# Cogito2012/3DFaceRecon

Hardware: AMD Instinct MI355X
Metric: faces/sec (3DMM decode+depth render), batch 64 @200x200 (higher is better)
Workload: dtype f32

## Files before the change

### 3dfacerecon_amd/_lib.py

```python
import ctypes
import hashlib
import os
import shutil
import subprocess
import sys
import threading
import types

_PKG_DIR = os.path.dirname(os.path.abspath(__file__))
_CSRC = os.path.join(_PKG_DIR, "csrc")
LIB_PATH = os.path.join(_PKG_DIR, "libfr_hotpath.so")
SOURCES = ["fr_capi.hip", "fr_render.hip", "fr_decode.hip", "fr_decode_q.hip", "fr_decode_bwd.hip", "fr_render_bwd.hip", "fr_render_nbwd.hip",
           "fr_render_tbwd.hip", "fr_sfs.hip", "fr_depth_normals.hip", "fr_geometry.hip", "fr_fine_losses.hip", "fr_depth_interp.hip",
           "fr_albedo_lse.hip", "fr_synth.hip", "fr_photo.hip", "fr_mesh.hip", "fr_coverage.hip", "fr_landmark.hip",
           "fr_landmark_solve.hip", "fr_landmark_contour.hip", "fr_photo_solve.hip", "fr_attr_interp.hip"]
HEADERS = [os.path.join(_CSRC, "fr_common.h"), os.path.join(_CSRC, "fr_decode_shared.h"), os.path.join(_CSRC, "fr_sfs_pinv.h"),
           os.path.join(_CSRC, "fr_owner_scatter.h"), os.path.join(_CSRC, "fr_shade.h"), os.path.join(_CSRC, "fr_landmark_shared.h"),
           os.path.join(_CSRC, "fr_point_weight.h"),
           os.path.join(_PKG_DIR, "..", "include", "fr_hotpath.h")]
HIPCC_FLAGS = ["--offload-arch=gfx950", "-O3", "-std=c++17", "-ffp-contract=off", "-fPIC", "-shared",
               "-mllvm", "-amdgpu-atomic-optimizer-strategy=None"]

FR_OK = 0
_ERR_NAMES = {-1: "invalid argument", -2: "workspace / packed buffer too small", -3: "HIP launch or runtime error",
# ... 147 lines not shown
    "fr_fine_losses_backward":                        "i:ppppiiippp",
    "fr_debug_fine_losses_geom":                      "v:iiiI",
    "fr_depth_interp_forward":                        "i:pippiiiiipp",
    "fr_depth_interp_backward_workspace_bytes":       "z:iiii",
    "fr_depth_interp_backward":                       "i:ppipppiiiiiipzp",
    "fr_debug_depth_interp_bwd_geom":                 "v:iiiiI",
    "fr_albedo_basis_bytes":                          "z:ii",
    "fr_albedo_basis_build":                          "i:ppiiipzp",
    "fr_sfs_lighting":                                "i:piiidpzp",
    "fr_albedo_lse_workspace_bytes":                  "z:iiii",
    "fr_albedo_lse_forward":                          "i:ppppppiiiiidppppzp",
    "fr_debug_albedo_lse_geom":                       "v:iiiiI",
    "fr_synth_params":                                "i:uuiiiifffpppppp",
    "fr_synth_texture":                               "i:pppiiipp",
    "fr_synth_shade":                                 "i:pppppiiiiffppp",
    "fr_synth_texture_backward_workspace_bytes":      "z:iii",
    "fr_synth_texture_backward":                      "i:ppiiippzp",
    "fr_photo_loss_state_bytes":                      "z:iii",
    "fr_photo_loss_forward":                          "i:ppppppiiiffppzp",
    "fr_photo_loss_backward":                         "i:ppppppppiiiffpppp",
    "fr_debug_photo_loss_geom":                       "v:iiiI",
    "fr_synth_light_rgb":                             "i:uuippp",
    "fr_synth_shade_rgb":                             "i:pppppiiiiffpppp",
    "fr_photo_loss_rgb_state_bytes":                  "z:iii",
    "fr_photo_loss_rgb_forward":                      "i:ppppppiiiffppzp",
    "fr_photo_loss_rgb_backward":                     "i:ppppppppiiiffpppp",
    "fr_debug_photo_loss_rgb_geom":                   "v:iiiI",
    "fr_albedo_basis_rgb_bytes":                      "z:ii",
    "fr_albedo_basis_rgb_build":                      "i:pppiiipzp",
    "fr_albedo_image_rgb":                            "i:pppiiiiipp",
    "fr_photo_solve_rgb_workspace_bytes":             "z:iii",
    "fr_photo_light_lse_rgb_forward":                 "i:ppppppiiiffdppppzp",
    "fr_albedo_lse_rgb_forward":                      "i:ppppppiiiiiffdppppzp",
    "fr_debug_photo_solve_rgb_geom":                  "v:iiiI",
    "fr_mesh_visible":                                "i:ppiiiiipp",
    "fr_mesh_lift":                                   "i:pippppiiiiipipp",
    "fr_mesh_vertex_normals":                         "i:pipppiiipip",
    "fr_attr_interp_forward":                         "i:pipippiiiiipp",
    "fr_attr_interp_backward":                        "i:ppipipppipiiiiiippp",
    "fr_mesh_vertex_normals_backward":                "i:pipipppiiippiip",
    "fr_debug_attr_interp_bwd_geom":                  "v:iiiiI",
    "fr_coverage_forward":                            "i:pippiiiiipp",
    "fr_coverage_backward_workspace_bytes":           "z:iiii",
    "fr_coverage_backward":                           "i:pppipppiiiiiipzp",
    "fr_debug_coverage_bwd_geom":                     "v:iiiiI",
    "fr_landmark_basis_bytes":                        "z:iii",
    "fr_landmark_basis_build":                        "i:ppppiiiipzp",
    "fr_landmark_forward":                            "i:ppzpppiiiiifppp",
    "fr_landmark_backward":                           "i:ppppzpppiiiiifppip",
    "fr_landmark_solve_workspace_bytes":              "z:iii",
    "fr_landmark_solve_step":                         "i:ppzppipppiiiiiifppppzp",
    "fr_landmark_contour_select":                     "i:ppzpppippipiiiiiiifppppp",
    "fr_debug_render_geom":                           "v:iiiiiI",
    "fr_debug_decode_bwd_geom":                       "v:iiiiI",
    "fr_debug_decode_geom":                           "i:iiiiiI",
    "fr_debug_decode_q_geom":                         "i:iiiiiiI",
    "fr_debug_decode_walk":                           "i:iiiiI",
    "fr_debug_pose_bwd_geom":                         "v:iiI",
    "fr_debug_render_bwd_geom":                       "v:iiiiI",
    "fr_debug_div3_sweep":                            "i:uupp",
    "fr_debug_clock_probe":                           "i:piip",
}
EXPORTS = list(SIGNATURES)


def bind(cdll, names=None):
    for name in (SIGNATURES if names is None else names):
        ret, args = SIGNATURES[name].split(":")
        fn = getattr(cdll, name)
        fn.restype = _CTYPE[ret]
        fn.argtypes = [_CTYPE[c] for c in args]
    return cdll


def lib():
    global _lib
    if _lib is None:
        with _lock:
            if _lib is None:
                import torch
                if is_stale():
                    compile()
                try:
                    L = bind(ctypes.CDLL(LIB_PATH))
                except OSError as e:
                    raise RuntimeError("fr_hotpath: cannot load %s (%s); run compile() -- there is no CPU fallback"
                                       % (LIB_PATH, e))
                want = src_hash()
                if want is not None and want.encode() not in L.fr_version():
                    raise RuntimeError("fr_hotpath: %s reports %r but the sources hash to %s: stale binary refused"
                                       % (LIB_PATH, L.fr_version(), want))
                _lib = L
    return _lib


DECODE_ARITH_Q30, DECODE_ARITH_F32 = 0, 1
_STATE = sys.modules.setdefault("_fr_hotpath_state", types.SimpleNamespace(decode_arith=None, q30_levels=7, option_epoch=0,
                                                                           pools={}))
_ARITH_ENV = {"q30": 7, "q30l7": 7, "q30l5": 5, "q30l4": 4}


def _torch_stream_key(dev):
    import torch
    return (dev.index if dev.index is not None else torch.cuda.current_device(), torch.cuda.current_stream(dev).cuda_stream,
            torch.cuda.is_current_stream_capturing())

# ... 159 lines not shown
```

### 3dfacerecon_amd/csrc/fr_capi.hip

```cpp
#include <atomic>
#include <mutex>

#include "fr_common.h"
#include "fr_landmark_shared.h"

namespace {
struct OptDesc {
    const char* name;
    int dflt;
    const char* word;
};
const OptDesc kOpts[fr::OPT_COUNT] = {
    {"FR_DECODE_IMPL", 0, "loop"}, {"FR_DECODE_WIDE", 1, nullptr}, {"FR_DECODE_NBW", 0, nullptr},
    {"FR_DECODE_WAVES", 16, nullptr}, {"FR_DECODE_NT", -1, nullptr}, {"FR_RESOLVE_OPT", 2, nullptr},
    {"FR_EMIT_FILTER", 3, nullptr}, {"FR_RENDER_IMPL", 0, "scan"}, {"FR_RESOLVE_BLOCK", 0, nullptr},
    {"FR_RENDER_ROWS", 0, nullptr}, {"FR_DECODE_STORE", 0, nullptr},
    {"FR_BWD_CHUNKS", 256, nullptr}, {"FR_BWD_CB", 0, nullptr}, {"FR_EMIT_ORDER", -1, nullptr},
    {"FR_Q30_SCHED", 0, nullptr}, {"FR_DECODE_CUS", 0, nullptr},
};
std::atomic<int> g_opt[fr::OPT_COUNT];
std::once_flag g_opt_once;
void opts_init() {
    for (int i = 0; i < fr::OPT_COUNT; i++) {
        int v = kOpts[i].dflt;
        const char* e = getenv(kOpts[i].name);
        if (e && *e) v = (kOpts[i].word && !strcmp(e, kOpts[i].word)) ? 1 : atoi(e);
        g_opt[i].store(v, std::memory_order_relaxed);
    }
}
int opt_index(const char* name) {
    if (!name) return -1;
    for (int i = 0; i < fr::OPT_COUNT; i++)
        if (!strcmp(name, kOpts[i].name)) return i;
    return -1;
}
}

int fr::opt(fr::Opt o) {
    std::call_once(g_opt_once, opts_init);
    return g_opt[o].load(std::memory_order_relaxed);
}

extern "C" {

int fr_set_option(const char* name, int value) {
    const int i = opt_index(name);
    if (i < 0) return FR_ERR_INVALID_ARG;
    std::call_once(g_opt_once, opts_init);
    g_opt[i].store(value, std::memory_order_relaxed);
    return FR_OK;
}

int fr_get_option(const char* name, int* value) {
    const int i = opt_index(name);
    if (i < 0 || !value) return FR_ERR_INVALID_ARG;
    *value = fr::opt((fr::Opt)i);
    return FR_OK;
}

#ifndef FR_SRC_HASH
#define FR_SRC_HASH "unhashed"
#endif
const char* fr_version(void) { return "fr_hotpath 0.4 (gfx950) src=" FR_SRC_HASH; }

const char* fr_strerror(int code) {
    switch (code) {
        case FR_OK: return "ok";
        case FR_ERR_INVALID_ARG: return "invalid argument";
        case FR_ERR_WORKSPACE: return "workspace / packed buffer too small";
        case FR_ERR_LAUNCH: return "HIP launch or runtime error";
        case FR_ERR_UNSUPPORTED: return "size not supported by the gfx950 kernels";
// ... 583 lines not shown
```

### 3dfacerecon_amd/csrc/fr_common.h

```cpp
#pragma once
#include <hip/hip_runtime.h>
#include <atomic>
#include <limits.h>
#include <stdint.h>
#include <stdlib.h>
#include <string.h>

#include "../../include/fr_hotpath.h"

namespace fr {

__device__ __forceinline__ float bg_depth() { return -99999999999999.0f; }

__device__ __forceinline__ int f2i_x86(float f) {
    return (f >= -2147483648.0f && f < 2147483648.0f) ? (int)f : INT_MIN;
}

__device__ __forceinline__ float mn(float a, float b) { return a < b ? a : b; }
__device__ __forceinline__ float mx(float a, float b) { return a > b ? a : b; }

__device__ __forceinline__ uint32_t f32_ord(float h) {
    uint32_t u = __float_as_uint(h);
    return (u & 0x80000000u) ? ~u : (u | 0x80000000u);
}
// ... 54 lines not shown

template <int K>
__device__ __forceinline__ double row_shl_f64(double v) {
    int lo = __double2loint(v), hi = __double2hiint(v);
    lo = __builtin_amdgcn_update_dpp(0, lo, 0x100 + K, 0xF, 0xF, true);
    hi = __builtin_amdgcn_update_dpp(0, hi, 0x100 + K, 0xF, 0xF, true);
    return __hiloint2double(hi, lo);
}
__device__ __forceinline__ double wave_tree_f64(double v) {
    v = v + __shfl_down(v, 32u, 64);
    v = v + __shfl_down(v, 16u, 64);
    v = v + row_shl_f64<8>(v);
    v = v + row_shl_f64<4>(v);
    v = v + row_shl_f64<2>(v);
    v = v + row_shl_f64<1>(v);
    return v;
}

}

typedef std::atomic<unsigned char> fr_lds_flags_t;
inline hipError_t fr_allow_full_lds(const void* kernel, fr_lds_flags_t* done ) {
    int dev = 0;
    hipError_t e = hipGetDevice(&dev);
    if (e != hipSuccess) return e;
    if (dev >= 0 && dev < 64 && done[dev].load(std::memory_order_acquire)) return hipSuccess;
    e = hipFuncSetAttribute(kernel, hipFuncAttributeMaxDynamicSharedMemorySize, 160 * 1024);
    if (e == hipSuccess && dev >= 0 && dev < 64) done[dev].store(1, std::memory_order_release);
    return e;
}

inline bool ws_ok(const void* p, size_t have, size_t need, size_t align) {
    return p && !((uintptr_t)p & (align - 1)) && have >= need;
}

namespace fr {
enum Opt {
    OPT_DECODE_IMPL,
    OPT_DECODE_WIDE,
    OPT_DECODE_NBW,
    OPT_DECODE_WAVES,
    OPT_DECODE_NT,
    OPT_RESOLVE_OPT,
    OPT_EMIT_FILTER,
    OPT_RENDER_IMPL,
    OPT_RESOLVE_BLOCK,
    OPT_RENDER_ROWS,
    OPT_DECODE_STORE,
    OPT_BWD_CHUNKS,
    OPT_BWD_CB,
    OPT_EMIT_ORDER,
    OPT_Q30_SCHED,
    OPT_DECODE_CUS,
    OPT_COUNT
};
int opt(Opt o);
}

int fr_launch_render_forward(const float* vertex, const float* tri, const float* texture, int B, int nver, int ntri,
                             int H, int W, int tex_batch, float* depth, float* tex_img, float* normal,
                             float* tri_ind, void* workspace, size_t ws_bytes, hipStream_t stream);
int fr_launch_render_forward_phases(const float* vertex, const float* tri, const float* texture, int B, int nver, int ntri,
                                    int H, int W, int tex_batch, float* depth, float* tex_img, float* normal,
                                    float* tri_ind, void* workspace, size_t ws_bytes, hipStream_t stream, int phases,
                                    long long vpitch = 0, int rows_hint = 0);
int fr_launch_rendering_layer(const float* vertex, const float* tri, const float* texture, const float* im_gray, int B,
                              int nver, int ntri, int H, int W, int tex_batch, float* net_in, float* depth_img,
                              float* depth, float* tri_ind, void* workspace, size_t ws_bytes, hipStream_t stream, int phases = 7,
                              long long vpitch = 0, int rows_hint = 0);
bool fr_rendering_layer_supported(int B, int nver, int ntri, int H, int W);
int fr_launch_render_backward(const float* depth_grad, const float* tri, const float* tri_ind, float* vertex_grad,
                              int B, int nver, int ntri, int H, int W, void* workspace, size_t ws_bytes,
                              hipStream_t stream);
struct FrPixelGrad {
    const float* g_depth;
    const float* g_depth_img;
    const float* g_net_input;
    const float* im_gray;
    const float* depth;
};
int fr_launch_render_backward_z(const FrPixelGrad& pg, const float* tri, const float* tri_ind, float* zplane, int zpitch,
                                int B, int nver, int ntri, int H, int W, void* workspace, size_t ws_bytes, hipStream_t stream);
size_t fr_render_backward_workspace_bytes_impl(int B, int H, int W);
size_t fr_render_workspace_bytes_impl(int B, int ntri, int H, int W);
size_t fr_packed_basis_bytes(int N, int n_shape, int n_exp);
int fr_launch_pack_basis(const float* mu, const float* pc_shape, const float* pc_exp, int N, int n_shape, int n_exp,
                         void* packed, hipStream_t stream);
int fr_launch_decode(const float* params, const void* packed, const float* R_override, int B, int N, int n_shape,
                     int n_exp, float im_size, float* vertex_proj, int pitch, hipStream_t stream);
int fr_launch_clock_probe(unsigned long long* out, int blocks, int iters, hipStream_t stream);
size_t fr_packed_q_bytes(int N, int n_shape, int n_exp);
bool fr_decode_q_supported(int n_shape, int n_exp);
int fr_launch_pack_q(const float* mu, const float* pc_shape, const float* pc_exp, int N, int n_shape, int n_exp,
                     void* qimage, hipStream_t stream);
int fr_launch_decode_q(const float* params, const void* qimage, const float* R_override, int B, int N, int n_shape,
                       int n_exp, float im_size, float* vertex_proj, int pitch, int levels, void* workspace, size_t ws_bytes,
                       hipStream_t stream);
bool fr_decode_q_levels_ok(int levels);
size_t fr_decode_q_workspace_bytes_impl(int n_shape, int n_exp);
int fr_device_cu_count();
int fr_decode_plan_cus();
size_t fr_decode_backward_workspace_impl(int N, int ns, int ne);
int fr_launch_decode_backward(const float* grad_vertex_proj, const float* params, const float* vertex_proj,
                              const float* pc_shape, const float* pc_exp, const float* R_override, int B, int N, int ns,
                              int ne, float im_size, float* grad_params, void* workspace, hipStream_t stream,
                              const void* packed_t = nullptr, const float* mu = nullptr, int zpitch = 0);
// ... 37 lines not shown
```

### 3dfacerecon_amd/csrc/fr_render.hip

```cpp
#include "fr_common.h"
#include <stddef.h>

namespace fr {

struct alignas(64) RenderArgs {
    const float* vertex;
    long long face_stride_b;
    long long vpitch_b;
    const int4* tri4_lane;
    long long tex_stride;
    int nseg;
    uint32_t nseg_magic;
    uint32_t nseg_shift;
    int emit_q, emit_r;
    int strips;
    float wm1, hm1;
    int use_filter;
    int nver, ntri;
    uint32_t rows_magic;
    const float* texture;
    float4* tritex_ws;
    const int4* tri4;
    uint4* recs;
    uint16_t* segoff;
// ... 285 lines not shown
            float4* t4 = reinterpret_cast<float4*>(txi) + 3 * (size_t)g;
            t4[0] = make_float4(o[0].tex[0], o[0].tex[1], o[0].tex[2], o[1].tex[0]);
            t4[1] = make_float4(o[1].tex[1], o[1].tex[2], o[2].tex[0], o[2].tex[1]);
            t4[2] = make_float4(o[2].tex[2], o[3].tex[0], o[3].tex[1], o[3].tex[2]);
            float4* n4 = reinterpret_cast<float4*>(nrm) + 3 * (size_t)g;
            n4[0] = make_float4(o[0].nrm[0], o[0].nrm[1], o[0].nrm[2], o[1].nrm[0]);
            n4[1] = make_float4(o[1].nrm[1], o[1].nrm[2], o[2].nrm[0], o[2].nrm[1]);
            n4[2] = make_float4(o[2].nrm[2], o[3].nrm[0], o[3].nrm[1], o[3].nrm[2]);
        }
    } else {
        for (int i = tid; i < npix; i += BLOCK) {
            PixelOut o = resolve_pixel(keys[i], vx, vy, vz, tri, tex, nver, ntri);
            dep[i] = o.depth;
            tin[i] = o.tind;
#pragma unroll
            for (int j = 0; j < 3; j++) {
                txi[3 * (size_t)i + j] = o.tex[j];
                nrm[3 * (size_t)i + j] = o.nrm[j];
            }
        }
    }
}

template <int BLOCK>
__global__ __launch_bounds__(BLOCK) void render_strip_kernel(RenderArgs a) {
    extern __shared__ __attribute__((aligned(16))) unsigned long long keys[];
    const int tid = threadIdx.x;
    const int bin = xcd_remap(blockIdx.x, gridDim.x);
    const int b = bin / a.strips;
    const int s = bin - b * a.strips;
    const int r0 = s * a.rows;
    const int r1 = min(a.H, r0 + a.rows);
    const int npix = (r1 - r0) * a.W;
    const unsigned long long KBG = bg_key();
    for (int i = tid; i < npix; i += BLOCK) keys[i] = KBG;
    __syncthreads();
    const float* __restrict__ vx = a.vertex + (size_t)b * 3 * a.vpitch;
    const float* __restrict__ vy = vx + a.vpitch;
    const float* __restrict__ vz = vy + a.vpitch;
    for (int t = tid; t < a.ntri; t += BLOCK)
        raster_triangle_into_strip(t, a.tri, vx, vy, vz, a.nver, a.ntri, a.H, a.W, r0, r1, keys);
    __syncthreads();
    write_strip<BLOCK, false>(a, b, r0, npix, keys, vx, vy, vz);
}

__device__ __forceinline__ float ld_off(const float* __restrict__ base, uint32_t idx) {
    return *reinterpret_cast<const float*>(reinterpret_cast<const char*>(base) + (size_t)(idx << 2));
}
__device__ __forceinline__ bool id_ok(float f, int n, int& p) {
    p = (int)f;
    return (f > -1.0f) && ((unsigned)p < (unsigned)n);
}

constexpr int TRI4_MAGIC = 0x46525435;
constexpr int PACK_TPT = 2;
constexpr int PACK_ACTIVE = SEG / PACK_TPT;
__device__ __forceinline__ int perm_local(int c, int j) {
    const int u = j >= PACK_ACTIVE ? 1 : 0, tid = j - u * PACK_ACTIVE;
    return c == 1 ? 2 * tid + u : j;
}
constexpr int PACK_NCAND = 2;
__global__ __launch_bounds__(256) void pack_tri_kernel(const float* __restrict__ tri, int nver, int ntri, int4* __restrict__ out,
                                                       int4* __restrict__ hdr, int4* __restrict__ outp, int force) {
    __shared__ int po[3][SEG];
    __shared__ unsigned char okf[SEG];
    __shared__ uint32_t cost[PACK_NCAND];
    const int seg = blockIdx.x, tid = threadIdx.x;
    if (seg == 0 && tid == 0) *hdr = make_int4(TRI4_MAGIC, nver, ntri, 0);
    if (tid < PACK_NCAND) cost[tid] = 0;
    for (int i = tid; i < SEG; i += 256) {
        const int t = seg * SEG + i;
        int p1 = 0, p2 = 0, p3 = 0;
        bool ok = false;
        if (t < ntri)
            ok = id_ok(tri[t], nver, p1) & id_ok(tri[(size_t)ntri + t], nver, p2) & id_ok(tri[2 * (size_t)ntri + t], nver, p3);
        const int4 e = ok ? make_int4(p1 << 2, p2 << 2, p3 << 2, 1) : make_int4(0, 0, 0, 0);
        out[t] = e;
        po[0][i] = e.x; po[1][i] = e.y; po[2][i] = e.z;
        okf[i] = ok ? 1 : 0;
    }
    __syncthreads();
    for (int j = tid; j < SEG; j += 256) {
        const int tl = j >= PACK_ACTIVE ? j - PACK_ACTIVE : j;
        if (tl & 15) {
#pragma unroll
            for (int c = 0; c < PACK_NCAND; c++) {
                const int ia = perm_local(c, j), ib = perm_local(c, j - 1);
                uint32_t br = 0;
#pragma unroll
                for (int k = 0; k < 3; k++) {
                    const int d = po[k][ia] - po[k][ib];
                    br += (d > 4 || d < -4) ? 1u : 0u;
                }
                if (br) atomicAdd(&cost[c], br);
            }
        }
    }
    __syncthreads();
    int c = 0;
    uint32_t best = cost[0];
#pragma unroll
    for (int k = 1; k < PACK_NCAND; k++)
        if (cost[k] < best) { best = cost[k]; c = k; }
    if (force >= 0 && force < PACK_NCAND) c = force;
    for (int j = tid; j < SEG; j += 256) {
        const int i = perm_local(c, j);
        outp[(size_t)seg * SEG + j] = make_int4(po[0][i], po[1][i], po[2][i], (int)okf[i] | (i << 1));
    }
}
__device__ __forceinline__ float ld_boff(const float* __restrict__ base, int boff) {
    return *reinterpret_cast<const float*>(reinterpret_cast<const char*>(base) + (size_t)(uint32_t)boff);
}
__device__ __forceinline__ uint32_t wave_inclusive_scan(uint32_t x) {
    x += (uint32_t)__builtin_amdgcn_update_dpp(0, (int)x, 0x111, 0xf, 0xf, true);
    x += (uint32_t)__builtin_amdgcn_update_dpp(0, (int)x, 0x112, 0xf, 0xf, true);
    x += (uint32_t)__builtin_amdgcn_update_dpp(0, (int)x, 0x114, 0xf, 0xf, true);
    x += (uint32_t)__builtin_amdgcn_update_dpp(0, (int)x, 0x118, 0xf, 0xf, true);
    x += (uint32_t)__builtin_amdgcn_update_dpp(0, (int)x, 0x142, 0xa, 0xf, false);
    x += (uint32_t)__builtin_amdgcn_update_dpp(0, (int)x, 0x143, 0xc, 0xf, false);
    return x;
}

struct NoEmitProbe {
    static constexpr int abl = 0;
    __device__ __forceinline__ void begin() {}
    template <int ID> __device__ __forceinline__ void stamp() {}
    __device__ __forceinline__ void finish(int) {}
};
__device__ __forceinline__ unsigned long long lanes(bool p) { return __builtin_amdgcn_ballot_w64(p); }
__device__ __forceinline__ bool lane_of(unsigned long long m) { return __builtin_amdgcn_inverse_ballot_w64(m); }
constexpr int EMIT_BLOCK = 256;
constexpr int TPT = 2;
constexpr int EMIT_ACTIVE = SEG / TPT;

constexpr size_t EMIT_LDS_QA = 0;
constexpr size_t EMIT_LDS_QB = EMIT_LDS_QA + SEG * sizeof(float4);
constexpr size_t EMIT_LDS_QD = EMIT_LDS_QB + SEG * sizeof(float4);
constexpr size_t EMIT_LDS_CNT = EMIT_LDS_QD + SEG * sizeof(uint2);
constexpr size_t EMIT_LDS_QN2 = EMIT_LDS_CNT + OFF_STRIDE * 4;
constexpr size_t EMIT_LDS_BYTES = EMIT_LDS_QN2 + 8;
static_assert(EMIT_LDS_BYTES == 20424 && 8 * EMIT_LDS_BYTES <= 160 * 1024, "eight emit workgroups per CU");

template <class PR>
__device__ __forceinline__ void emit_body(const RenderArgs& a, const int lid, unsigned char* lds, PR& pr) {
    float4* const qa = reinterpret_cast<float4*>(lds + EMIT_LDS_QA);
    float4* const qb = reinterpret_cast<float4*>(lds + EMIT_LDS_QB);
    uint2* const qd = reinterpret_cast<uint2*>(lds + EMIT_LDS_QD);
    uint32_t* const cnt = reinterpret_cast<uint32_t*>(lds + EMIT_LDS_CNT);
    unsigned long long& qn2 = *reinterpret_cast<unsigned long long*>(lds + EMIT_LDS_QN2);
    const int tid = threadIdx.x;
    if constexpr (PR::abl == 1) return;
    const int b = (int)(__umulhi((uint32_t)lid << 1, a.nseg_magic) >> a.nseg_shift);
    const int seg = lid - b * a.nseg;
    const int S = a.strips;
    if (tid < 2 * S) cnt[tid] = 0;
    if (tid == 0) qn2 = 0ull;

    const int nver = a.nver, ntri = a.ntri;
    const char* const vbase = reinterpret_cast<const char*>(a.vertex) + (unsigned long long)(uint32_t)b * (unsigned long long)a.face_stride_b;
    const float* __restrict__ vx = reinterpret_cast<const float*>(vbase);
    const float* __restrict__ vy = reinterpret_cast<const float*>(vbase + a.vpitch_b);
    const float* __restrict__ vz = reinterpret_cast<const float*>(vbase + 2 * a.vpitch_b);

    {
        unsigned long long surv[TPT], single[TPT], valid[TPT];
        int4 e[TPT];
        float x1[TPT], x2[TPT], x3[TPT], y1[TPT], y2[TPT], y3[TPT], z1[TPT], z2[TPT], z3[TPT];
        const int4* __restrict__ tri4p = a.tri4_lane + (size_t)(uint32_t)seg * SEG;
        int tl[TPT];
#pragma unroll
        for (int u = 0; u < TPT; u++) {
            e[u] = *reinterpret_cast<const int4*>(reinterpret_cast<const char*>(tri4p) + (size_t)((uint32_t)min(u * EMIT_ACTIVE + tid, SEG - 1) << 4));
            tl[u] = e[u].w >> 1;
        }
        const int4 hdr = a.tri4_lane[-1];
        if constexpr (PR::abl == 2) {
            if (e[0].x + e[1].y == 0x7fffffff) qd[tid].x = 1;
            return;
        }
#pragma unroll
        for (int u = 0; u < TPT; u++) {
            x1[u] = ld_boff(vx, e[u].x); x2[u] = ld_boff(vx, e[u].y); x3[u] = ld_boff(vx, e[u].z);
            y1[u] = ld_boff(vy, e[u].x); y2[u] = ld_boff(vy, e[u].y); y3[u] = ld_boff(vy, e[u].z);
            z1[u] = ld_boff(vz, e[u].x); z2[u] = ld_boff(vz, e[u].y); z3[u] = ld_boff(vz, e[u].z);
        }
        if constexpr (PR::abl == 3) {
            float acc = 0.f;
#pragma unroll
            for (int u = 0; u < TPT; u++) acc += ((x1[u] + x2[u]) + x3[u]) + ((y1[u] + y2[u]) + y3[u]) + ((z1[u] + z2[u]) + z3[u]);
            if (acc == 1.2345e30f) qd[tid].x = 1;
            return;
        }
        asm volatile("s_waitcnt lgkmcnt(0)\n\ts_barrier" ::: "memory");
        pr.template stamp<0>();
        const bool table_ok = (hdr.x == TRI4_MAGIC) & (hdr.y == nver) & (hdr.z == ntri);
        const unsigned long long owners = lanes(tid < EMIT_ACTIVE) & (table_ok ? ~0ull : 0ull);
        const unsigned long long precull = (a.use_filter & 2) ? ~0ull : 0ull;
#pragma unroll
        for (int u = 0; u < TPT; u++) {
            valid[u] = owners & lanes((e[u].w & 1) != 0);
            const float fx0 = ceilf(fminf(fminf(x1[u], x2[u]), x3[u])), fx1 = floorf(fmaxf(fmaxf(x1[u], x2[u]), x3[u]));
            const float fy0 = ceilf(fminf(fminf(y1[u], y2[u]), y3[u])), fy1 = floorf(fmaxf(fmaxf(y1[u], y2[u]), y3[u]));
            surv[u] = valid[u] & lanes(fx0 >= 0.0f) & lanes(fy0 >= 0.0f) & lanes(fx1 <= a.wm1) & lanes(fy1 <= a.hm1) &
                      lanes(!(fx1 < fx0)) & lanes(!(fy1 < fy0));
            single[u] = lanes(fx0 == fx1) & lanes(fy0 == fy1);
            {
                const float v0x = x3[u] - x1[u], v0y = y3[u] - y1[u], v1x = x2[u] - x1[u], v1y = y2[u] - y1[u];
                const float D = __builtin_fmaf(v0x, v1y, -(v0y * v1x));
                const float M0 = fmaxf(fmaxf(fabsf(v0x), fabsf(v0y)), fmaxf(fabsf(v1x), fabsf(v1y)));
                const float S = M0 * M0;
                const float v2x = fx0 - x1[u], v2y = fy0 - y1[u];
                const float A = __builtin_fmaf(v2x, v1y, -(v2y * v1x)), Bq = __builtin_fmaf(v0x, v2y, -(v0y * v2x)), C = (D - A) - Bq;
                const unsigned long long certain = lanes(M0 < 1073741824.0f) & lanes(M0 > 9.094947017729282e-13f) &
                                                   lanes(fabsf(D) >= 0.00390625f * S) &
                                                   lanes(fminf(fminf(fabsf(A), fabsf(Bq)), fabsf(C)) >= 1.52587890625e-05f * S);
                const unsigned long long dpos = lanes(D > 0.0f);
                const unsigned long long in = (dpos & lanes(fminf(fminf(A, Bq), C) > 0.0f)) | (~dpos & lanes(fmaxf(fmaxf(A, Bq), C) < 0.0f));
                surv[u] &= ~(precull & single[u] & certain & ~in);
            }
        }
        pr.template stamp<1>();
        static_assert(TPT == 2, "compaction below is written for two triangles per thread");
        const unsigned long long ms0 = surv[0] & single[0], ms1 = surv[1] & single[1];
        const unsigned long long mm0 = surv[0] & ~single[0], mm1 = surv[1] & ~single[1];
        const uint32_t cs0 = (uint32_t)__popcll(ms0), cs1 = (uint32_t)__popcll(ms1);
        const uint32_t cm0 = (uint32_t)__popcll(mm0), cm1 = (uint32_t)__popcll(mm1);
        unsigned long long wb = 0;
        if ((tid & 63) == 0 && (cs0 + cs1 + cm0 + cm1))
            wb = atomicAdd(&qn2, ((unsigned long long)(cm0 + cm1) << 32) | (unsigned long long)(cs0 + cs1));
        const uint32_t fbase = (uint32_t)__builtin_amdgcn_readfirstlane((int)(uint32_t)wb);
        const uint32_t bbase = (uint32_t)__builtin_amdgcn_readfirstlane((int)(uint32_t)(wb >> 32));
#pragma unroll
        for (int u = 0; u < TPT; u++) {
            if (lane_of(surv[u])) {
                const unsigned long long ms = u ? ms1 : ms0, mm = u ? mm1 : mm0;
                const uint32_t rs = __builtin_amdgcn_mbcnt_hi((uint32_t)(ms >> 32), __builtin_amdgcn_mbcnt_lo((uint32_t)ms, 0u));
                const uint32_t rm = __builtin_amdgcn_mbcnt_hi((uint32_t)(mm >> 32), __builtin_amdgcn_mbcnt_lo((uint32_t)mm, 0u));
                const uint32_t slot = lane_of(single[u]) ? fbase + (u ? cs0 : 0u) + rs
                                                : (uint32_t)(SEG - 1) - (bbase + (u ? cm0 : 0u) + rm);
                qa[slot] = make_float4(x1[u], y1[u], x2[u], y2[u]);
                qb[slot] = make_float4(x3[u], y3[u], z1[u], z2[u]);
                qd[slot] = make_uint2(__float_as_uint(z3[u]), (uint32_t)tl[u]);
            }
        }
        if (a.tex_stride == 0 && b == 0) {
#pragma unroll
            for (int u = 0; u < TPT; u++) {
                if (lane_of(valid[u])) {
                    float tm[3];
#pragma unroll
                    for (int j = 0; j < 3; j++) {
                        const float* tj = a.texture + (size_t)j * nver;
                        tm[j] = div3((ld_boff(tj, e[u].x) + ld_boff(tj, e[u].y)) + ld_boff(tj, e[u].z));
                    }
                    a.tritex_ws[seg * SEG + tl[u]] = make_float4(tm[0], tm[1], tm[2], 0.0f);
                }
            }
        }
    }
    pr.template stamp<2>();
    if constexpr (PR::abl == 5) return;
    __syncthreads();
    pr.template stamp<3>();

    const unsigned long long q2 = qn2;
    const int nqf = (int)(uint32_t)q2, nq = nqf + (int)(uint32_t)(q2 >> 32);
    for (int qi = tid; qi < nq; qi += EMIT_BLOCK) {
        const int sl = qi < nqf ? qi : SEG - 1 - (qi - nqf);
        const float4 A4 = qa[sl], B4 = qb[sl];
        const uint2 D2 = qd[sl];
        const float x1 = A4.x, y1 = A4.y, x2 = A4.z, y2 = A4.w, x3 = B4.x, y3 = B4.y;
        const float z1 = B4.z, z2 = B4.w, z3 = __uint_as_float(D2.x);
        bool emit = false;
        int bucket = 0;
        uint4 rec = make_uint4(0, 0, 0, 0);
        float4 nrm4 = make_float4(0.f, 0.f, 0.f, 0.f);
        float h = div3((z1 + z2) + z3);
        h = h + 0.0f;
        const int t = seg * SEG + (int)D2.y;
        if (h > bg_depth()) {
            const int x_min = (int)ceilf(fminf(fminf(x1, x2), x3)), x_max = (int)floorf(fmaxf(fmaxf(x1, x2), x3));
            const int y_min = (int)ceilf(fminf(fminf(y1, y2), y3)), y_max = (int)floorf(fmaxf(fmaxf(y1, y2), y3));
            const unsigned long long key = make_key(h, t);
            rec.x = (uint32_t)key;
            rec.y = (uint32_t)(key >> 32);
            rec.z = (uint32_t)x_min | ((uint32_t)y_min << 16);
            const int s0 = a.rows_magic ? (int)__umulhi((uint32_t)y_min, a.rows_magic) : y_min;
            const int s1 = a.rows_magic ? (int)__umulhi((uint32_t)y_max, a.rows_magic) : y_max;
            if (x_max - x_min < SMALL_W && y_max - y_min < SMALL_H) {
                const float v0x = x3 - x1, v0y = y3 - y1, v1x = x2 - x1, v1y = y2 - y1;
                const float D = __builtin_fmaf(v0x, v1y, -(v0y * v1x));
                const float M0 = fmaxf(fmaxf(fabsf(v0x), fabsf(v0y)), fmaxf(fabsf(v1x), fabsf(v1y)));
                const float S = M0 * M0;
                const float tm = 1.52587890625e-05f * S;
                const bool tri_ok = (a.use_filter & 1) && (M0 < 1073741824.0f) && (M0 > 9.094947017729282e-13f) &&
                                    (fabsf(D) >= 0.00390625f * S);
                const bool dpos = D > 0.0f;
                const int bw = x_max - x_min + 1, npx = bw * (y_max - y_min + 1);
                int dx = 0, bit = 0, yy = y_min;
                uint32_t m = 0, unsure = 0;
#pragma clang loop unroll(disable)
                for (int k = 0; k < npx; k++) {
                    const float v2x = (float)(x_min + dx) - x1, v2y = (float)yy - y1;
                    const float A = __builtin_fmaf(v2x, v1y, -(v2y * v1x)), Bq = __builtin_fmaf(v0x, v2y, -(v0y * v2x)), C = (D - A) - Bq;
                    const bool certain = tri_ok && fminf(fminf(fabsf(A), fabsf(Bq)), fabsf(C)) >= tm;
                    const bool in = dpos ? fminf(fminf(A, Bq), C) > 0.0f : fmaxf(fmaxf(A, Bq), C) < 0.0f;
// ... 618 lines not shown
    a.wm1 = (float)(W - 1);
    a.hm1 = (float)(H - 1);
    a.resolve_opt = opt(OPT_RESOLVE_OPT);
    a.use_filter = opt(OPT_EMIT_FILTER);
    a.rows_magic = g.rows > 1 ? (uint32_t)((0x100000000ull + (unsigned)g.rows - 1) / (unsigned)g.rows) : 0u;
    a.tri4 = nullptr; a.tri4_lane = nullptr;
    a.nseg_magic = 0; a.nseg_shift = 0; a.emit_q = 0; a.emit_r = 0;
    const bool binned = g.binned_ok && ntri > 0 && opt(OPT_RENDER_IMPL) != 1;
    *binned_out = binned;
    if (fused && !binned) return FR_ERR_UNSUPPORTED;
    if (!binned) return FR_OK;
    if (ws_bytes < g.recs_bytes + g.segoff_bytes + 2 * g.nrm_bytes + g.tri4_bytes || !workspace ||
        ((uintptr_t)workspace & 15))
        return FR_ERR_WORKSPACE;
    char* wsp = reinterpret_cast<char*>(workspace);
    a.recs = reinterpret_cast<uint4*>(wsp);
    a.segoff = reinterpret_cast<uint16_t*>(wsp + g.recs_bytes + g.nrm_bytes);
    a.tritex_ws = reinterpret_cast<float4*>(wsp + g.recs_bytes + g.segoff_bytes + g.nrm_bytes);
    a.tri4 = reinterpret_cast<int4*>(wsp + g.recs_bytes + g.segoff_bytes + 2 * g.nrm_bytes);
    a.tri4_lane = a.tri4 + ((size_t)g.nseg * SEG + 1);
    const long long nlid = (long long)B * g.nseg;
    if (nlid > 0 && !emit_index_magic(nlid, g.nseg, &a.nseg_magic, &a.nseg_shift)) return FR_ERR_UNSUPPORTED;
    a.emit_q = (int)(nlid >> 3); a.emit_r = (int)(nlid & 7);
    return FR_OK;
}

static int launch_render_impl(const float* vertex, const float* tri, const float* texture, int B, int nver, int ntri, int H,
                              int W, int tex_batch, float* depth, float* tex_img, float* normal, float* tri_ind,
                              const float* im_gray, float* net_in, float* depth_img, void* workspace, size_t ws_bytes,
                              hipStream_t stream, int phases, long long vpitch, int rows_hint) {
    using namespace fr;
    const bool fused = net_in != nullptr;
    constexpr int BLOCK = 1024;
    if (nver == 0) ntri = 0;
    RenderArgs a;
    RenderGeom g;
    bool binned = false;
    if (rows_hint > 0 && !(render_geom(B, ntri, H, W, rows_hint).binned_ok && render_geom(B, ntri, H, W).binned_ok)) rows_hint = 0;
    const int prc = prepare_render(vertex, tri, texture, B, nver, ntri, H, W, tex_batch, depth, tex_img, normal, tri_ind, im_gray,
                                   net_in, depth_img, workspace, ws_bytes, vpitch, a, g, &binned, rows_hint > 0 ? rows_hint : -1);
    if (prc != FR_OK) return prc;
    const long long nbins = (long long)B * g.strips;
    if (!binned) {
        if (!(phases & 2)) return FR_OK;
        static fr_lds_flags_t lds_ok[64];
        if (fr_allow_full_lds(reinterpret_cast<const void*>(&render_strip_kernel<BLOCK>), lds_ok) != hipSuccess)
            return FR_ERR_LAUNCH;
        hipLaunchKernelGGL(render_strip_kernel<BLOCK>, dim3((unsigned)nbins), dim3(BLOCK), g.lds, stream, a);
        return hipGetLastError() == hipSuccess ? FR_OK : FR_ERR_LAUNCH;
    }
    if (phases & 4) {
        int4* tri4 = const_cast<int4*>(a.tri4);
        hipLaunchKernelGGL(pack_tri_kernel, dim3((unsigned)g.nseg), dim3(256), 0, stream, tri, nver, ntri, tri4,
                           tri4 + (size_t)g.nseg * SEG, tri4 + (size_t)g.nseg * SEG + 1, opt(OPT_EMIT_ORDER));
    }
    if (phases & 1)
        hipLaunchKernelGGL(raster_emit_kernel<NoEmitProbe>, dim3((unsigned)((long long)B * g.nseg)), dim3(EMIT_BLOCK), 0, stream, a);
    if (!(phases & 2)) return hipGetLastError() == hipSuccess ? FR_OK : FR_ERR_LAUNCH;
    const int rblk = opt(OPT_RESOLVE_BLOCK) > 0 ? opt(OPT_RESOLVE_BLOCK) : (g.lds <= 32 * 1024 ? 256 : 512);
    int rc;
    if (rblk == 1024)
        rc = fused ? launch_resolve<1024, true>(a, nbins, g.lds, stream) : launch_resolve<1024, false>(a, nbins, g.lds, stream);
    else if (rblk == 512)
        rc = fused ? launch_resolve<512, true>(a, nbins, g.lds, stream) : launch_resolve<512, false>(a, nbins, g.lds, stream);
    else
        rc = fused ? launch_resolve<256, true>(a, nbins, g.lds, stream) : launch_resolve<256, false>(a, nbins, g.lds, stream);
    if (rc != FR_OK) return rc;
    return hipGetLastError() == hipSuccess ? FR_OK : FR_ERR_LAUNCH;
}
```

### include/fr_hotpath.h

```cpp
#ifndef FR_HOTPATH_H_
#define FR_HOTPATH_H_

#include <stddef.h>

#ifdef __cplusplus
extern "C" {
#endif

#define FR_OK 0
#define FR_ERR_INVALID_ARG (-1)
#define FR_ERR_WORKSPACE (-2)
#define FR_ERR_LAUNCH (-3)
#define FR_ERR_UNSUPPORTED (-4)

#define FR_N_POSE 7

const char* fr_version(void);
const char* fr_strerror(int code);

int fr_set_option(const char* name, int value);
int fr_get_option(const char* name, int* value);

size_t fr_render_depth_workspace_bytes(int B, int nver, int ntri, int H, int W);

// ... 245 lines not shown
                    void* stream);
int fr_mesh_lift(const float* vertex, int vertex_pitch, const float* tri_ind, const unsigned char* visible, const float* fine_depth,
                 const float* coarse_depth, int B, int nver, int ntri, int H, int W, float* vertex_out, int out_pitch,
                 unsigned char* state, void* stream);
int fr_mesh_vertex_normals(const float* vertex, int vertex_pitch, const float* tri, const int* adj_start, const int* adj_tri, int B,
                           int nver, int ntri, float* normal, int out_pitch, void* stream);

int fr_attr_interp_forward(const float* vertex, int vertex_pitch, const float* attr, int attr_pitch, const float* tri,
                           const float* tri_ind, int B, int nver, int ntri, int H, int W, float* out, void* stream);
int fr_attr_interp_backward(const float* grad, const float* vertex, int vertex_pitch, const float* attr, int attr_pitch,
                            const float* tri, const float* tri_ind, float* attr_grad, int attr_accumulate, float* vertex_grad,
                            int vertex_accumulate, int B, int nver, int ntri, int H, int W, int* records, unsigned int* partial,
                            void* stream);
int fr_mesh_vertex_normals_backward(const float* normal_grad, int grad_pitch, const float* vertex, int vertex_pitch, const float* tri,
                                    const int* adj_start, const int* adj_tri, int B, int nver, int ntri, double* h,
                                    float* vertex_grad, int out_pitch, int accumulate, void* stream);

void fr_debug_attr_interp_bwd_geom(int B, int nver, int H, int W, int* out);

int fr_coverage_forward(const float* vertex, int vertex_pitch, const float* tri, const float* tri_ind, int B, int nver, int ntri,
                        int H, int W, float* cov, void* stream);
size_t fr_coverage_backward_workspace_bytes(int B, int nver, int H, int W);
int fr_coverage_backward(const float* cov_grad, const float* cov, const float* vertex, int vertex_pitch, const float* tri,
                         const float* tri_ind, float* vertex_grad, int B, int nver, int ntri, int H, int W, int accumulate,
                         void* workspace, size_t ws_bytes, void* stream);

void fr_debug_coverage_bwd_geom(int B, int nver, int H, int W, int* out);

size_t fr_landmark_basis_bytes(int K, int n_shape, int n_exp);
int fr_landmark_basis_build(const float* mu, const float* pc_shape, const float* pc_exp, const int* idx, int N, int n_shape,
                            int n_exp, int K, void* lbasis, size_t bytes, void* stream);
int fr_landmark_forward(const float* params, const void* lbasis, size_t lbasis_bytes, const float* R_override, const float* target,
                        const float* weight, int weight_batch, int B, int K, int n_shape, int n_exp, float im_size, float* points,
                        double* sse, void* stream);
int fr_landmark_backward(const float* grad_points, const double* grad_sse, const float* params, const void* lbasis,
                         size_t lbasis_bytes, const float* R_override, const float* target, const float* weight, int weight_batch,
                         int B, int K, int n_shape, int n_exp, float im_size, float* grad_params, float* grad_R, int pose_grad,
                         void* stream);

size_t fr_landmark_solve_workspace_bytes(int B, int n_shape, int n_exp);
int fr_landmark_solve_step(const float* params, const void* lbasis, size_t lbasis_bytes, const float* target, const float* weight,
                           int weight_batch, const float* ridge, const float* center, const double* damp, int pose_mask, int fit_coef,
                           int B, int K, int n_shape, int n_exp, float im_size, double* delta, double* cost, int* ok, void* workspace,
                           size_t workspace_bytes, void* stream);

int fr_landmark_contour_select(const float* params, const void* lbasis, size_t lbasis_bytes, const float* R_override,
                               const float* fixed_target, const float* fixed_weight, int fixed_weight_batch, const float* line_target,
                               const float* line_weight, int line_weight_batch, const float* line_dir, int rule, int B, int Kf, int C,
                               int M, int n_shape, int n_exp, float im_size, int* sel, float* line_points, float* target, float* weight,
                               void* stream);

void fr_debug_render_geom(int B, int ntri, int H, int W, int rows_override, int* out);

void fr_debug_decode_bwd_geom(int nbatch, int N, int n_shape, int n_exp, int* out);

int fr_debug_decode_geom(int B, int N, int n_shape, int n_exp, int cus, int* out);

int fr_debug_decode_q_geom(int B, int N, int n_shape, int n_exp, int levels, int cus, int* out);

int fr_debug_decode_walk(int tiles, int waves, int halves, int grid, int* visits);

void fr_debug_pose_bwd_geom(int B, int N, int* out);

void fr_debug_render_bwd_geom(int B, int nver, int H, int W, int* out);

int fr_debug_div3_sweep(unsigned long long first, unsigned long long count, unsigned long long* mismatches,
                        void* hip_stream);

int fr_debug_clock_probe(unsigned long long* ticks, int blocks, int iters, void* hip_stream);

#ifdef __cplusplus
}
#endif
#endif
```

Before: 670,100.

## Share vertices between paired triangles in raster emit via packed shared entries

The triangle packer now detects wavefronts where each lane's two triangles share an edge (quad strips) and encodes a compact shared entry holding four vertex offsets. When a wave is shared, the emit kernel does one int4 load instead of two and takes the third vertex of adjacent triangles from the neighbouring lane with DPP row shifts rather than loading it from global memory. The aim is fewer index and vertex gathers in the emit phase. The cost is extra branching, a more complex pack kernel, and a dependence on mesh topology. A host debug entry point for inspecting lane classes is added, and the path is on by default behind FR_EMIT_SHARE.

```diff
diff --git a/3dfacerecon_amd/_lib.py b/3dfacerecon_amd/_lib.py
--- a/3dfacerecon_amd/_lib.py
+++ b/3dfacerecon_amd/_lib.py
@@ -223,6 +223,7 @@
     "fr_landmark_solve_step":                         "i:ppzppipppiiiiiifppppzp",
     "fr_landmark_contour_select":                     "i:ppzpppippipiiiiiiifppppp",
     "fr_debug_render_geom":                           "v:iiiiiI",
+    "fr_debug_emit_lanes":                            "i:piiiI",
     "fr_debug_decode_bwd_geom":                       "v:iiiiI",
     "fr_debug_decode_geom":                           "i:iiiiiI",
     "fr_debug_decode_q_geom":                         "i:iiiiiiI",
diff --git a/3dfacerecon_amd/csrc/fr_capi.hip b/3dfacerecon_amd/csrc/fr_capi.hip
--- a/3dfacerecon_amd/csrc/fr_capi.hip
+++ b/3dfacerecon_amd/csrc/fr_capi.hip
@@ -16,7 +16,7 @@
     {"FR_EMIT_FILTER", 3, nullptr}, {"FR_RENDER_IMPL", 0, "scan"}, {"FR_RESOLVE_BLOCK", 0, nullptr},
     {"FR_RENDER_ROWS", 0, nullptr}, {"FR_DECODE_STORE", 0, nullptr},
     {"FR_BWD_CHUNKS", 256, nullptr}, {"FR_BWD_CB", 0, nullptr}, {"FR_EMIT_ORDER", -1, nullptr},
-    {"FR_Q30_SCHED", 0, nullptr}, {"FR_DECODE_CUS", 0, nullptr},
+    {"FR_Q30_SCHED", 0, nullptr}, {"FR_DECODE_CUS", 0, nullptr}, {"FR_EMIT_SHARE", 1, nullptr},
 };
 std::atomic<int> g_opt[fr::OPT_COUNT];
 std::once_flag g_opt_once;
diff --git a/3dfacerecon_amd/csrc/fr_common.h b/3dfacerecon_amd/csrc/fr_common.h
--- a/3dfacerecon_amd/csrc/fr_common.h
+++ b/3dfacerecon_amd/csrc/fr_common.h
@@ -130,6 +130,7 @@
     OPT_EMIT_ORDER,
     OPT_Q30_SCHED,
     OPT_DECODE_CUS,
+    OPT_EMIT_SHARE,
     OPT_COUNT
 };
 int opt(Opt o);
diff --git a/3dfacerecon_amd/csrc/fr_render.hip b/3dfacerecon_amd/csrc/fr_render.hip
--- a/3dfacerecon_amd/csrc/fr_render.hip
+++ b/3dfacerecon_amd/csrc/fr_render.hip
@@ -361,64 +361,141 @@
     return (f > -1.0f) && ((unsigned)p < (unsigned)n);
 }
 
-constexpr int TRI4_MAGIC = 0x46525435;
+constexpr int TRI4_MAGIC = 0x46525436;
 constexpr int PACK_TPT = 2;
 constexpr int PACK_ACTIVE = SEG / PACK_TPT;
-__device__ __forceinline__ int perm_local(int c, int j) {
+__host__ __device__ __forceinline__ bool id_ok_hd(float f, int n, int& p) {
+#if defined(__HIP_DEVICE_COMPILE__)
+    return id_ok(f, n, p);
+#else
+    const bool ok = (f > -1.0f) && ((double)f < (double)n);
+    p = ok ? (int)f : 0;
+    return ok;
+#endif
+}
+__host__ __device__ __forceinline__ bool tri_offsets(const float* __restrict__ tri, int nver, int ntri, int t, int* o) {
+    int p1 = 0, p2 = 0, p3 = 0;
+    bool ok = false;
+    if (t < ntri)
+        ok = id_ok_hd(tri[t], nver, p1) & id_ok_hd(tri[(size_t)ntri + t], nver, p2) & id_ok_hd(tri[2 * (size_t)ntri + t], nver, p3);
+    o[0] = ok ? p1 << 2 : 0; o[1] = ok ? p2 << 2 : 0; o[2] = ok ? p3 << 2 : 0;
+    return ok;
+}
+__host__ __device__ __forceinline__ int perm_local(int c, int j) {
     const int u = j >= PACK_ACTIVE ? 1 : 0, tid = j - u * PACK_ACTIVE;
     return c == 1 ? 2 * tid + u : j;
 }
 constexpr int PACK_NCAND = 2;
+__host__ __device__ __forceinline__ uint32_t pack_pos_cost(const int (*po)[SEG], int c, int j) {
+    const int tl = j >= PACK_ACTIVE ? j - PACK_ACTIVE : j;
+    if (!(tl & 15)) return 0;
+    const int ia = perm_local(c, j), ib = perm_local(c, j - 1);
+    uint32_t br = 0;
+    for (int k = 0; k < 3; k++) {
+        const int d = po[k][ia] - po[k][ib];
+        br += (d > 4 || d < -4) ? 1u : 0u;
+    }
+    return br;
+}
+constexpr int EMIT_LANE_PAIR = 1, EMIT_LANE_NEXT = 2, EMIT_LANE_NEXT_ROW = 4, EMIT_LANE_SHARED = 8, EMIT_LANE_ORDER_SHIFT = 4;
+__host__ __device__ __forceinline__ bool emit_lane_pair(const int (*po)[SEG], const unsigned char* okf, int c, int tid) {
+    const int i0 = perm_local(c, tid), i1 = perm_local(c, PACK_ACTIVE + tid);
+    return okf[i0] && okf[i1] && po[0][i1] == po[2][i0] && po[1][i1] == po[1][i0];
+}
+__host__ __device__ __forceinline__ int emit_lane_class(const int (*po)[SEG], const unsigned char* okf, int c, int tid) {
+    if (tid >= PACK_ACTIVE || !emit_lane_pair(po, okf, c, tid)) return 0;
+    int f = EMIT_LANE_PAIR;
+    if (tid + 1 < PACK_ACTIVE && ((tid + 1) & 63) && emit_lane_pair(po, okf, c, tid + 1)) {
+        const int i0 = perm_local(c, tid), i1 = perm_local(c, PACK_ACTIVE + tid), n0 = perm_local(c, tid + 1);
+        if (po[2][i0] == po[0][n0] && po[2][i1] == po[1][n0]) f |= EMIT_LANE_NEXT | (((tid + 1) & 15) ? EMIT_LANE_NEXT_ROW : 0);
+    }
+    return f;
+}
+constexpr int SHARE_ENTRY = 1, SHARE_NEXT = 2;
+__host__ __device__ __forceinline__ int pack_choose_order(const uint32_t* cost, int force) {
+    int c = 0;
+    uint32_t best = cost[0];
+    for (int k = 1; k < PACK_NCAND; k++)
+        if (cost[k] < best) { best = cost[k]; c = k; }
+    if (force >= 0 && force < PACK_NCAND) c = force;
+    return c;
+}
 __global__ __launch_bounds__(256) void pack_tri_kernel(const float* __restrict__ tri, int nver, int ntri, int4* __restrict__ out,
-                                                       int4* __restrict__ hdr, int4* __restrict__ outp, int force) {
+                                                       int4* __restrict__ hdr, int4* __restrict__ outp, int force, int share) {
     __shared__ int po[3][SEG];
     __shared__ unsigned char okf[SEG];
     __shared__ uint32_t cost[PACK_NCAND];
+    __shared__ uint32_t notpair[4];
     const int seg = blockIdx.x, tid = threadIdx.x;
     if (seg == 0 && tid == 0) *hdr = make_int4(TRI4_MAGIC, nver, ntri, 0);
     if (tid < PACK_NCAND) cost[tid] = 0;
+    if (tid < 4) notpair[tid] = 0;
     for (int i = tid; i < SEG; i += 256) {
         const int t = seg * SEG + i;
-        int p1 = 0, p2 = 0, p3 = 0;
-        bool ok = false;
-        if (t < ntri)
-            ok = id_ok(tri[t], nver, p1) & id_ok(tri[(size_t)ntri + t], nver, p2) & id_ok(tri[2 * (size_t)ntri + t], nver, p3);
-        const int4 e = ok ? make_int4(p1 << 2, p2 << 2, p3 << 2, 1) : make_int4(0, 0, 0, 0);
-        out[t] = e;
-        po[0][i] = e.x; po[1][i] = e.y; po[2][i] = e.z;
+        int o[3];
+        const bool ok = tri_offsets(tri, nver, ntri, t, o);
+        out[t] = make_int4(o[0], o[1], o[2], ok ? 1 : 0);
+        po[0][i] = o[0]; po[1][i] = o[1]; po[2][i] = o[2];
         okf[i] = ok ? 1 : 0;
     }
     __syncthreads();
     for (int j = tid; j < SEG; j += 256) {
-        const int tl = j >= PACK_ACTIVE ? j - PACK_ACTIVE : j;
-        if (tl & 15) {
-#pragma unroll
-            for (int c = 0; c < PACK_NCAND; c++) {
-                const int ia = perm_local(c, j), ib = perm_local(c, j - 1);
-                uint32_t br = 0;
-#pragma unroll
-                for (int k = 0; k < 3; k++) {
-                    const int d = po[k][ia] - po[k][ib];
-                    br += (d > 4 || d < -4) ? 1u : 0u;
-                }
-                if (br) atomicAdd(&cost[c], br);
-            }
+#pragma unroll
+        for (int c = 0; c < PACK_NCAND; c++) {
+            const uint32_t br = pack_pos_cost(po, c, j);
+            if (br) atomicAdd(&cost[c], br);
         }
     }
     __syncthreads();
-    int c = 0;
-    uint32_t best = cost[0];
-#pragma unroll
-    for (int k = 1; k < PACK_NCAND; k++)
-        if (cost[k] < best) { best = cost[k]; c = k; }
-    if (force >= 0 && force < PACK_NCAND) c = force;
+    const int c = pack_choose_order(cost, force);
+    const int cls = emit_lane_class(po, okf, c, tid);
+    if (tid < PACK_ACTIVE && !(cls & EMIT_LANE_PAIR)) atomicOr(&notpair[tid >> 6], 1u);
+    __syncthreads();
     for (int j = tid; j < SEG; j += 256) {
         const int i = perm_local(c, j);
-        outp[(size_t)seg * SEG + j] = make_int4(po[0][i], po[1][i], po[2][i], (int)okf[i] | (i << 1));
-    }
-}
+        int4 e = make_int4(po[0][i], po[1][i], po[2][i], (int)okf[i] | (i << 1));
+        if (share && c == 1 && j < PACK_ACTIVE && !notpair[j >> 6])
+            e = make_int4(e.x | SHARE_ENTRY | ((cls & EMIT_LANE_NEXT_ROW) ? SHARE_NEXT : 0), e.y, e.z, po[2][perm_local(c, PACK_ACTIVE + j)]);
+        outp[(size_t)seg * SEG + j] = e;
+    }
+}
+}
+
+extern "C" int fr_debug_emit_lanes(const float* tri, int nver, int ntri, int order, int* out) {
+    using namespace fr;
+    if (!out || nver < 0 || ntri < 0 || (ntri > 0 && !tri)) return FR_ERR_INVALID_ARG;
+    const int nseg = (ntri + SEG - 1) / SEG;
+    static thread_local int po[3][SEG];
+    static thread_local unsigned char okf[SEG];
+    for (int seg = 0; seg < nseg; seg++) {
+        for (int i = 0; i < SEG; i++) {
+            int o[3];
+            okf[i] = tri_offsets(tri, nver, ntri, seg * SEG + i, o) ? 1 : 0;
+            po[0][i] = o[0]; po[1][i] = o[1]; po[2][i] = o[2];
+        }
+        uint32_t cost[PACK_NCAND] = {};
+        for (int j = 0; j < SEG; j++)
+            for (int c = 0; c < PACK_NCAND; c++) cost[c] += pack_pos_cost(po, c, j);
+        const int c = pack_choose_order(cost, order);
+        int* o = out + (size_t)seg * 256;
+        for (int w = 0; w < 4; w++) {
+            bool all = c == 1;
+            for (int tid = 64 * w; tid < 64 * w + 64; tid++) {
+                o[tid] = emit_lane_class(po, okf, c, tid) | (c << EMIT_LANE_ORDER_SHIFT);
+                if (tid < PACK_ACTIVE && !(o[tid] & EMIT_LANE_PAIR)) all = false;
+            }
+            for (int tid = 64 * w; all && tid < 64 * w + 64 && tid < PACK_ACTIVE; tid++) o[tid] |= EMIT_LANE_SHARED;
+        }
+    }
+    return nseg;
+}
+
+namespace fr {
 __device__ __forceinline__ float ld_boff(const float* __restrict__ base, int boff) {
     return *reinterpret_cast<const float*>(reinterpret_cast<const char*>(base) + (size_t)(uint32_t)boff);
+}
+__device__ __forceinline__ float row_shl1(float x) {
+    return __int_as_float(__builtin_amdgcn_update_dpp(0, __float_as_int(x), 0x101, 0xf, 0xf, true));
 }
 __device__ __forceinline__ uint32_t wave_inclusive_scan(uint32_t x) {
     x += (uint32_t)__builtin_amdgcn_update_dpp(0, (int)x, 0x111, 0xf, 0xf, true);
@@ -473,41 +550,76 @@
 
     {
         unsigned long long surv[TPT], single[TPT], valid[TPT];
-        int4 e[TPT];
+        int o1[TPT], o2[TPT], o3[TPT];
         float x1[TPT], x2[TPT], x3[TPT], y1[TPT], y2[TPT], y3[TPT], z1[TPT], z2[TPT], z3[TPT];
         const int4* __restrict__ tri4p = a.tri4_lane + (size_t)(uint32_t)seg * SEG;
         int tl[TPT];
-#pragma unroll
-        for (int u = 0; u < TPT; u++) {
-            e[u] = *reinterpret_cast<const int4*>(reinterpret_cast<const char*>(tri4p) + (size_t)((uint32_t)min(u * EMIT_ACTIVE + tid, SEG - 1) << 4));
-            tl[u] = e[u].w >> 1;
-        }
+        const int4 e0 = *reinterpret_cast<const int4*>(reinterpret_cast<const char*>(tri4p) + (size_t)((uint32_t)min(tid, EMIT_ACTIVE - 1) << 4));
         const int4 hdr = a.tri4_lane[-1];
-        if constexpr (PR::abl == 2) {
-            if (e[0].x + e[1].y == 0x7fffffff) qd[tid].x = 1;
-            return;
-        }
-#pragma unroll
-        for (int u = 0; u < TPT; u++) {
-            x1[u] = ld_boff(vx, e[u].x); x2[u] = ld_boff(vx, e[u].y); x3[u] = ld_boff(vx, e[u].z);
-            y1[u] = ld_boff(vy, e[u].x); y2[u] = ld_boff(vy, e[u].y); y3[u] = ld_boff(vy, e[u].z);
-            z1[u] = ld_boff(vz, e[u].x); z2[u] = ld_boff(vz, e[u].y); z3[u] = ld_boff(vz, e[u].z);
-        }
-        if constexpr (PR::abl == 3) {
-            float acc = 0.f;
-#pragma unroll
-            for (int u = 0; u < TPT; u++) acc += ((x1[u] + x2[u]) + x3[u]) + ((y1[u] + y2[u]) + y3[u]) + ((z1[u] + z2[u]) + z3[u]);
-            if (acc == 1.2345e30f) qd[tid].x = 1;
-            return;
-        }
-        asm volatile("s_waitcnt lgkmcnt(0)\n\ts_barrier" ::: "memory");
+        const bool shared = (__builtin_amdgcn_readfirstlane(e0.x) & SHARE_ENTRY) != 0;
+        unsigned long long vbit[TPT];
+        if (shared) {
+            o1[0] = e0.x & ~(SHARE_ENTRY | SHARE_NEXT); o2[0] = e0.y; o3[0] = e0.z;
+            o1[1] = e0.z; o2[1] = e0.y; o3[1] = e0.w;
+            const unsigned long long nxm = lanes((e0.x & SHARE_NEXT) != 0);
+            tl[0] = 2 * tid; tl[1] = 2 * tid + 1;
+            vbit[0] = vbit[1] = ~0ull;
+            if constexpr (PR::abl == 2) {
+                if (e0.x + e0.y == 0x7fffffff) qd[tid].x = 1;
+                return;
+            }
+            x1[0] = ld_boff(vx, o1[0]); y1[0] = ld_boff(vy, o1[0]); z1[0] = ld_boff(vz, o1[0]);
+            x2[0] = ld_boff(vx, o2[0]); y2[0] = ld_boff(vy, o2[0]); z2[0] = ld_boff(vz, o2[0]);
+            if (!lane_of(nxm)) {
+                x3[0] = ld_boff(vx, o3[0]); y3[0] = ld_boff(vy, o3[0]); z3[0] = ld_boff(vz, o3[0]);
+                x3[1] = ld_boff(vx, o3[1]); y3[1] = ld_boff(vy, o3[1]); z3[1] = ld_boff(vz, o3[1]);
+            }
+            if constexpr (PR::abl == 3) {
+                float acc = ((x1[0] + x2[0]) + (y1[0] + y2[0])) + (z1[0] + z2[0]);
+                if (!lane_of(nxm)) acc += ((x3[0] + x3[1]) + (y3[0] + y3[1])) + (z3[0] + z3[1]);
+                if (acc == 1.2345e30f) qd[tid].x = 1;
+                return;
+            }
+            asm volatile("s_waitcnt lgkmcnt(0)\n\ts_barrier" ::: "memory");
+            const float ax = row_shl1(x1[0]), ay = row_shl1(y1[0]), az = row_shl1(z1[0]);
+            const float bx = row_shl1(x2[0]), by = row_shl1(y2[0]), bz = row_shl1(z2[0]);
+            if (lane_of(nxm)) {
+                x3[0] = ax; y3[0] = ay; z3[0] = az;
+                x3[1] = bx; y3[1] = by; z3[1] = bz;
+            }
+            x1[1] = x3[0]; y1[1] = y3[0]; z1[1] = z3[0];
+            x2[1] = x2[0]; y2[1] = y2[0]; z2[1] = z2[0];
+        } else {
+            const int4 e1 = *reinterpret_cast<const int4*>(reinterpret_cast<const char*>(tri4p) + (size_t)((uint32_t)min(EMIT_ACTIVE + tid, SEG - 1) << 4));
+            o1[0] = e0.x; o2[0] = e0.y; o3[0] = e0.z; tl[0] = e0.w >> 1;
+            o1[1] = e1.x; o2[1] = e1.y; o3[1] = e1.z; tl[1] = e1.w >> 1;
+            vbit[0] = lanes((e0.w & 1) != 0); vbit[1] = lanes((e1.w & 1) != 0);
+            if constexpr (PR::abl == 2) {
+                if (e0.x + e1.y == 0x7fffffff) qd[tid].x = 1;
+                return;
+            }
+#pragma unroll
+            for (int u = 0; u < TPT; u++) {
+                x1[u] = ld_boff(vx, o1[u]); x2[u] = ld_boff(vx, o2[u]); x3[u] = ld_boff(vx, o3[u]);
+                y1[u] = ld_boff(vy, o1[u]); y2[u] = ld_boff(vy, o2[u]); y3[u] = ld_boff(vy, o3[u]);
+                z1[u] = ld_boff(vz, o1[u]); z2[u] = ld_boff(vz, o2[u]); z3[u] = ld_boff(vz, o3[u]);
+            }
+            if constexpr (PR::abl == 3) {
+                float acc = 0.f;
+#pragma unroll
+                for (int u = 0; u < TPT; u++) acc += ((x1[u] + x2[u]) + x3[u]) + ((y1[u] + y2[u]) + y3[u]) + ((z1[u] + z2[u]) + z3[u]);
+                if (acc == 1.2345e30f) qd[tid].x = 1;
+                return;
+            }
+            asm volatile("s_waitcnt lgkmcnt(0)\n\ts_barrier" ::: "memory");
+        }
         pr.template stamp<0>();
         const bool table_ok = (hdr.x == TRI4_MAGIC) & (hdr.y == nver) & (hdr.z == ntri);
         const unsigned long long owners = lanes(tid < EMIT_ACTIVE) & (table_ok ? ~0ull : 0ull);
         const unsigned long long precull = (a.use_filter & 2) ? ~0ull : 0ull;
 #pragma unroll
         for (int u = 0; u < TPT; u++) {
-            valid[u] = owners & lanes((e[u].w & 1) != 0);
+            valid[u] = owners & vbit[u];
             const float fx0 = ceilf(fminf(fminf(x1[u], x2[u]), x3[u])), fx1 = floorf(fmaxf(fmaxf(x1[u], x2[u]), x3[u]));
             const float fy0 = ceilf(fminf(fminf(y1[u], y2[u]), y3[u])), fy1 = floorf(fmaxf(fmaxf(y1[u], y2[u]), y3[u]));
             surv[u] = valid[u] & lanes(fx0 >= 0.0f) & lanes(fy0 >= 0.0f) & lanes(fx1 <= a.wm1) & lanes(fy1 <= a.hm1) &
@@ -560,7 +672,7 @@
 #pragma unroll
                     for (int j = 0; j < 3; j++) {
                         const float* tj = a.texture + (size_t)j * nver;
-                        tm[j] = div3((ld_boff(tj, e[u].x) + ld_boff(tj, e[u].y)) + ld_boff(tj, e[u].z));
+                        tm[j] = div3((ld_boff(tj, o1[u]) + ld_boff(tj, o2[u])) + ld_boff(tj, o3[u]));
                     }
                     a.tritex_ws[seg * SEG + tl[u]] = make_float4(tm[0], tm[1], tm[2], 0.0f);
                 }
@@ -1285,7 +1397,7 @@
     if (phases & 4) {
         int4* tri4 = const_cast<int4*>(a.tri4);
         hipLaunchKernelGGL(pack_tri_kernel, dim3((unsigned)g.nseg), dim3(256), 0, stream, tri, nver, ntri, tri4,
-                           tri4 + (size_t)g.nseg * SEG, tri4 + (size_t)g.nseg * SEG + 1, opt(OPT_EMIT_ORDER));
+                           tri4 + (size_t)g.nseg * SEG, tri4 + (size_t)g.nseg * SEG + 1, opt(OPT_EMIT_ORDER), opt(OPT_EMIT_SHARE));
     }
     if (phases & 1)
         hipLaunchKernelGGL(raster_emit_kernel<NoEmitProbe>, dim3((unsigned)((long long)B * g.nseg)), dim3(EMIT_BLOCK), 0, stream, a);
diff --git a/include/fr_hotpath.h b/include/fr_hotpath.h
--- a/include/fr_hotpath.h
+++ b/include/fr_hotpath.h
@@ -321,6 +321,8 @@
 
 void fr_debug_render_geom(int B, int ntri, int H, int W, int rows_override, int* out);
 
+int fr_debug_emit_lanes(const float* tri, int nver, int ntri, int order, int* out);
+
 void fr_debug_decode_bwd_geom(int nbatch, int N, int n_shape, int n_exp, int* out);
 
 int fr_debug_decode_geom(int B, int N, int n_shape, int n_exp, int cus, int* out);
```

Measured after the change: 669,000. About the same (-0.2%).
